# mikel-brostrom/boxmot

Measured on NVIDIA H100. Metric: tracker.update() frames/sec at 256 dets/frame, higher is better.
Workload: dtype bf16x3

## Files before the change

boxmot_b200/csrc/reid_tc.cuh:

```cuda
#pragma once
#include "wgmma.cuh"

namespace bmb {
namespace tcx {

typedef __nv_bfloat16 bf16;

__device__ __forceinline__ int tc_chunk_count(const int* d_n, int off, int cap) {
    int n = *d_n - off;
    n = n < 0 ? 0 : n;
    return n > cap ? cap : n;
}
using um::mbar_arrive;

__global__ void k_maxpool_planes(const float* __restrict__ in, int H, int W, int C, const int* __restrict__ d_n, int off,
                                 int cap, bf16* __restrict__ out_hi, bf16* __restrict__ out_lo) {
    const int n_crops = tc_chunk_count(d_n, off, cap);
    const int OH = H / 2, OW = W / 2, C8 = C / 8;
    const size_t total = (size_t)n_crops * C8 * OH * OW;
    for (size_t e = (size_t)blockIdx.x * blockDim.x + threadIdx.x; e < total; e += (size_t)gridDim.x * blockDim.x) {
        const int ox = (int)(e % OW);
        size_t r = e / OW;
        const int oy = (int)(r % OH); r /= OH;
        const int c8 = (int)(r % C8);
// ... 334 lines not shown
        }
        if (last && CP > CR) {
            constexpr int PP = (CP - CR) / 8;
            static_assert((CP - CR) % 8 == 0, "channel padding must be whole planes");
            for (int e = threadIdx.x; e < PP * rows_lv * W; e += 256) {
                const int pl = e / (rows_lv * W), r = e - pl * (rows_lv * W);
                const size_t o = (((size_t)n * (4 * C8) + br * C8 + CR / 8 + pl) * H + ya) * W + r;
                reinterpret_cast<uint4*>(a.y_hi)[o] = make_uint4(0u, 0u, 0u, 0u);
                reinterpret_cast<uint4*>(a.y_lo)[o] = make_uint4(0u, 0u, 0u, 0u);
            }
        }
        um::fence_async_smem();
        __syncthreads();
        TCK();
    }
#ifdef BMB_TC_CLOCKS
    if (threadIdx.x == 0 && blockIdx.x == 1 && n == 5) {
        printf("chain CP%d W%d br%d: setup %lld tma %lld |", CP, W, br, ck[1] - ck[0], ck[2] - ck[1]);
        for (int i = 2; i + 3 < nck + 1 && i + 3 <= 23; i += 3)
            printf(" wait %lld mma %lld dw %lld |", ck[i + 1] - ck[i], ck[i + 2] - ck[i + 1], ck[i + 3] - ck[i + 2]);
        printf(" total %lld\n", ck[nck - 1] - ck[0]);
    }
#endif
    if (threadIdx.x < act)
        *reinterpret_cast<float4*>(sP + (threadIdx.x / C4) * CR + (threadIdx.x % C4) * 4) = psum;
    __syncthreads();
    for (int c = threadIdx.x; c < CP; c += 256) {
        float s = 0.f;
        if (c < CR)
            for (int g = 0; g < n_grp; ++g) s += sP[g * CR + c];
        a.sums[br][((size_t)n * gridDim.x + tile) * CP + c] = s;
    }
    __threadfence();
    __syncthreads();
    __shared__ int s_last;
    __shared__ float s_mean[128], s_hid[16], s_gate[128];
    if (threadIdx.x == 0) {
        const int total = (int)gridDim.x * 4;
        const int prev = atomicAdd(a.gate.arrivals + n, 1);
        s_last = prev == total - 1;
        if (s_last) a.gate.arrivals[n] = 0;
    }
    __syncthreads();
    if (s_last) {
        __threadfence();
        gates_fold<256>(a.gate, n, s_mean, s_hid, s_gate);
    }
}

#ifndef BMB_S2_NS
#define BMB_S2_NS 0
#endif
#ifndef BMB_S3_R
#define BMB_S3_R 16
#endif
#ifndef BMB_S3_NS
#define BMB_S3_NS 0
#endif
#ifndef BMB_S4_NS
#define BMB_S4_NS 0
#endif
#define BMB_CHAIN_S2 16, 16, 32, 16, BMB_S2_NS
#define BMB_CHAIN_S3 32, 24, 16, BMB_S3_R, BMB_S3_NS
#define BMB_CHAIN_S4 32, 32, 8, 16, BMB_S4_NS
template <int CP, int CR, int W, int R, int NSPLIT>
inline cudaError_t chain_prepare() {
    return cudaFuncSetAttribute(k_chain_tc<CP, CR, W, R, NSPLIT>, cudaFuncAttributeMaxDynamicSharedMemorySize, (int)ChainGeom<CP, CR, W, R>::SMEM);
}
template <int CP, int CR, int W, int R, int NSPLIT>
inline void chain_launch(const ChainTcArgs& a, int tiles, int crops, const int* d_n, int off, cudaStream_t st) {
    k_chain_tc<CP, CR, W, R, NSPLIT><<<dim3(tiles, 4, crops), 256, ChainGeom<CP, CR, W, R>::SMEM, st>>>(a, d_n, off, crops);
}
template <int CP, int CR, int W, int R, int NSPLIT>
constexpr int chain_rows() { return R; }

constexpr int GEMM_THREADS = 288;

struct GemmTcArgs {
    CUtensorMap map_hi[2], map_lo[2];
    int src_planes[2];
    int src_kc[2];
    int n_src;
    int rows_per_tile;
    int tiles_per_crop, tiles_per_cta;
    int n_stage;
    const bf16* b_packed;
    int K8;
    int N, NP;
    const float* bias;
    int relu;
    const bf16* bfold;
    int midp, HW;
    int slot_bytes;
    bf16* out_hi; bf16* out_lo;
    float* out_f32;
    int pool;
    int pool2;
    int W;
    const bf16* b2_packed;
    const float* bias2;
    int N2, NP2;
    bf16* out2_hi; bf16* out2_lo;
    const float* head_w;
    const float* head_b;
    int head_feat;
};
struct GemmHeadIO {
    const CropDesc* crops;
    float* out;
    int out_ld;
};

struct GemmSmem {
    size_t b, b2, ring, a2, f, gate, total;
};
inline GemmSmem gemm_smem_layout(int K8, int NP, int NP2, int n_stage, bool tail, bool pool, int slot_bytes, bool pool2 = false) {
    GemmSmem s{};
    size_t o = 0;
    s.b = o; o += (size_t)K8 * 2 * NP * 16;
    s.b2 = o; if (tail) o += (size_t)(NP / 8) * 2 * NP2 * 16;
    o = (o + 127) & ~(size_t)127;
    s.ring = o; o += (size_t)n_stage * slot_bytes;
    s.a2 = o;
    if (tail) {
        size_t a2 = (size_t)2 * (NP / 8) * 128 * 16;
        if (pool2) a2 = a2 > (size_t)128 * (NP2 + 4) * 4 ? a2 : (size_t)128 * (NP2 + 4) * 4;
        o += a2;
    }
    s.f = pool2 ? s.a2 : o;
    if (pool) o += (size_t)128 * (NP + 4) * 4;
    s.gate = o; o += 4 * 32 * 4 + 64;
    s.total = o + 128;
    return s;
}

enum GemmMode { GM_PLAIN, GM_POOL, GM_TAIL, GM_TAIL_POOL2, GM_HEAD };

template <int NP, int NP2, int MODE>
constexpr int gemm_min_ctas() {
    return NP == 128 || ((MODE == GM_TAIL || MODE == GM_TAIL_POOL2) && NP >= 96) ? 1 : 2;
}

template <int NP, int NP2, int MODE>
__global__ void __launch_bounds__(GEMM_THREADS, (gemm_min_ctas<NP, NP2, MODE>()))
    k_gemm_tc(const __grid_constant__ GemmTcArgs a, const int* __restrict__ d_n, int off, int cap, const GemmSmem L, const GemmHeadIO hio) {
    constexpr bool tail = MODE == GM_TAIL || MODE == GM_TAIL_POOL2, pool = MODE == GM_POOL, pool2 = MODE == GM_TAIL_POOL2;
    static_assert(NP % 16 == 0 && NP >= 16 && NP <= 128, "NP: 16 .. 128 output channels");
    static_assert(tail ? (NP2 % 16 == 0 && NP2 >= 16 && NP2 <= 128) : NP2 == 0, "NP2: the tail's output channels");
    constexpr int NACC = (NP2 > NP ? NP2 : NP) / 2;
    const int n = blockIdx.y;
    if (n >= tc_chunk_count(d_n, off, cap)) return;
    extern __shared__ __align__(128) unsigned char smem[];
    __shared__ __align__(8) uint64_t bar_full[4], bar_empty[4], bar_w;
    const int warp = threadIdx.x >> 5, lane = threadIdx.x & 31;
    const int tile0 = blockIdx.x * a.tiles_per_cta;
    const int tile1 = min(tile0 + a.tiles_per_cta, a.tiles_per_crop);
    unsigned char* sB = smem + L.b;
    unsigned char* sB2 = smem + L.b2;
    unsigned char* sRing = smem + L.ring;
    unsigned char* sA2 = smem + L.a2;
    float* sF = reinterpret_cast<float*>(smem + L.f);

    if (threadIdx.x == 0) {
        for (int i = 0; i < a.n_stage; ++i) { um::mbar_init(&bar_full[i], 1); um::mbar_init(&bar_empty[i], 2); }
        um::mbar_init(&bar_w, 1);
        um::fence_mbar_init();
    }
    __syncthreads();

    if (warp == 8) {
        if (lane == 0) {
            {
                const uint32_t first = (uint32_t)((a.bfold ? 4 * a.midp : 0) / 8) * 2u * NP * 16u, total = (uint32_t)a.K8 * 2u * NP * 16u;
                const uint32_t b2 = tail ? (uint32_t)(NP / 8) * 2u * NP2 * 16u : 0u;
                um::mbar_expect_tx(&bar_w, total + b2);
                if (first) um::bulk_g2s(sB, reinterpret_cast<const unsigned char*>(a.bfold) + (size_t)n * first, first, &bar_w);
                if (total > first) um::bulk_g2s(sB + first, reinterpret_cast<const unsigned char*>(a.b_packed) + first, total - first, &bar_w);
                if (b2) um::bulk_g2s(sB2, a.b2_packed, b2, &bar_w);
            }
            uint32_t it = 0;
            for (int tile = tile0; tile < tile1; ++tile) {
                for (int s = 0; s < a.n_src; ++s) {
                    const int kc = a.src_kc[s];
                    for (int p0 = 0; p0 < a.src_planes[s]; p0 += kc, ++it) {
                        const uint32_t slot = it % (uint32_t)a.n_stage, ph = (it / (uint32_t)a.n_stage) & 1u;
                        um::mbar_wait(&bar_empty[slot], ph ^ 1u);
                        unsigned char* dst = sRing + (size_t)slot * a.slot_bytes;
                        um::mbar_expect_tx(&bar_full[slot], (uint32_t)kc * 128u * 16u * 2u);
                        um::tma_load_4d(dst, &a.map_hi[s], 0, tile * 2, p0, n, &bar_full[slot]);
                        um::tma_load_4d(dst + a.slot_bytes / 2, &a.map_lo[s], 0, tile * 2, p0, n, &bar_full[slot]);
                    }
                }
            }
        }
        return;
    }

    const int et = threadIdx.x;
    const int wg = warp >> 2;
    const int row = wg * 64 + (warp & 3) * 16 + (lane >> 2);
    const int cq = 2 * (lane & 3);
    const uint32_t lbo_b = 2u * NP * 16u, lo_off = (uint32_t)NP * 16u;
    um::mbar_wait(&bar_w, 0);
    float acc[NACC];
    uint32_t it = 0;
    for (int tile = tile0; tile < tile1; ++tile) {
        uint32_t kplane = 0, first = 1;
        uint32_t held = 0;
        for (int s = 0; s < a.n_src; ++s) {
            const int kc = a.src_kc[s];
            for (int p0 = 0; p0 < a.src_planes[s]; p0 += kc, ++it) {
                const uint32_t slot = it % (uint32_t)a.n_stage, ph = (it / (uint32_t)a.n_stage) & 1u;
                um::mbar_wait(&bar_full[slot], ph);
                const uint32_t ah = um::smem_u32(sRing + (size_t)slot * a.slot_bytes) + (uint32_t)wg * 1024u, al = ah + a.slot_bytes / 2;
                for (int ks = 0; ks < kc / 2; ++ks) {
                    const uint32_t bb = um::smem_u32(sB) + (kplane + 2 * ks) * lbo_b;
                    const uint64_t xh = um::make_desc(ah + ks * 2 * 2048u, 2048u, 128), xl = um::make_desc(al + ks * 2 * 2048u, 2048u, 128);
                    um::wg_fence();
                    um::mma<NP, false>(acc, xh, bb, lbo_b, 128, first ? 0u : 1u);
                    um::mma<NP, false>(acc, xl, bb, lbo_b, 128, 1u);
                    um::mma<NP, false>(acc, xh, bb + lo_off, lbo_b, 128, 1u);
                    first = 0;
                    um::wg_commit();
                    um::wg_wait<1>();
                    if (ks == 0 && kplane > 0 && (et & 127) == 0) mbar_arrive(&bar_empty[held]);
                }
                held = slot;
                kplane += kc;
            }
        }
        um::wg_wait<0>();
        um::wg_fence_acc<NACC>(acc);
        if ((et & 127) == 0) mbar_arrive(&bar_empty[held]);
        if constexpr (MODE == GM_HEAD) {
            um::bar_sync(1, 256);
            float* part = reinterpret_cast<float*>(sRing);
            float* pooled = part + 8 * NP;
            float* red = pooled + NP;
            float* feat = red + 8;
#pragma unroll
            for (int i = 0; i < NP / 8; ++i) {
                const int c = 8 * i + cq;
                const float2 b = *reinterpret_cast<const float2*>(a.bias + c);
                float o0 = fmaxf(acc[4 * i] + b.x, 0.f) + fmaxf(acc[4 * i + 2] + b.x, 0.f);
                float o1 = fmaxf(acc[4 * i + 1] + b.y, 0.f) + fmaxf(acc[4 * i + 3] + b.y, 0.f);
#pragma unroll
                for (int sh = 4; sh < 32; sh <<= 1) {
                    o0 += __shfl_xor_sync(0xffffffffu, o0, sh);
                    o1 += __shfl_xor_sync(0xffffffffu, o1, sh);
                }
                if (lane < 4) *reinterpret_cast<float2*>(part + warp * NP + c) = make_float2(o0, o1);
            }
            um::bar_sync(1, 256);
            for (int c = et; c < NP; c += 256)
                pooled[c] = (((part[c] + part[NP + c]) + (part[2 * NP + c] + part[3 * NP + c])) +
                             ((part[4 * NP + c] + part[5 * NP + c]) + (part[6 * NP + c] + part[7 * NP + c]))) / 128.f;
            um::bar_sync(1, 256);
            const int FEAT = a.head_feat, C = a.N;
            float sq = 0.f;
            for (int f = et; f < FEAT; f += 256) {
                float t[8] = {0.f, 0.f, 0.f, 0.f, 0.f, 0.f, 0.f, 0.f};
                int c = 0;
                for (; c + 8 <= C; c += 8) {
#pragma unroll
                    for (int u = 0; u < 8; ++u) t[u] = fmaf(pooled[c + u], a.head_w[(size_t)(c + u) * FEAT + f], t[u]);
                }
                for (; c < C; ++c) t[0] = fmaf(pooled[c], a.head_w[(size_t)c * FEAT + f], t[0]);
                float sv = a.head_b[f] + (((t[0] + t[1]) + (t[2] + t[3])) + ((t[4] + t[5]) + (t[6] + t[7])));
                sv = fmaxf(sv, 0.f);
                feat[f] = sv;
                sq = fmaf(sv, sv, sq);
            }
#pragma unroll
            for (int sh = 16; sh > 0; sh >>= 1) sq += __shfl_xor_sync(0xffffffffu, sq, sh);
            if (lane == 0) red[warp] = sq;
            um::bar_sync(1, 256);
            float tot = 0.f;
            for (int w = 0; w < 8; ++w) tot += red[w];
            const float nrm = sqrtf(tot);
            float* dst = hio.out + (size_t)hio.crops[off + n].out_row * hio.out_ld;
            for (int f = et; f < FEAT; f += 256) dst[f] = feat[f] / nrm;
            um::bar_sync(1, 256);
        } else {
#pragma unroll
            for (int i = 0; i < NP / 8; ++i) {
                const int c = 8 * i + cq;
                const float2 b = *reinterpret_cast<const float2*>(a.bias + c);
#pragma unroll
                for (int h = 0; h < 2; ++h) {
                    const int m = row + 8 * h, px = tile * 128 + m;
                    float o0 = acc[4 * i + 2 * h] + b.x, o1 = acc[4 * i + 2 * h + 1] + b.y;
                    if (a.relu) { o0 = fmaxf(o0, 0.f); o1 = fmaxf(o1, 0.f); }
                    if (a.out_f32) {
                        float* dst = a.out_f32 + ((size_t)n * a.HW + px) * a.N + c;
                        if (c + 1 < a.N) *reinterpret_cast<float2*>(dst) = make_float2(o0, o1);
                        else if (c < a.N) dst[0] = o0;
                    }
                    if constexpr (pool) {
                        *reinterpret_cast<float2*>(sF + (size_t)m * (NP + 4) + c) = make_float2(o0, o1);
                    } else if (a.out_hi || tail) {
                        uint32_t hv, lv;
                        um::split2(o0, o1, hv, lv);
                        if (a.out_hi) {
                            const size_t e = (((size_t)n * (NP / 8) + i) * a.HW + px) * 4 + (lane & 3);
                            reinterpret_cast<uint32_t*>(a.out_hi)[e] = hv;
                            reinterpret_cast<uint32_t*>(a.out_lo)[e] = lv;
                        }
                        if constexpr (tail) {
                            *reinterpret_cast<uint32_t*>(sA2 + ((size_t)i * 128 + m) * 16 + (lane & 3) * 4) = hv;
                            *reinterpret_cast<uint32_t*>(sA2 + ((size_t)(NP / 8 + i) * 128 + m) * 16 + (lane & 3) * 4) = lv;
                        }
                    }
                }
            }
            auto pool_store = [&](const int NPx, bf16* o_hi, bf16* o_lo) {
                um::bar_sync(1, 256);
                const int Wt = a.W, OW = Wt / 2, OHt = a.rows_per_tile / 2;
                const int items = OHt * OW * (NPx / 8);
                const int OHW = a.HW / 4;
                for (int e = et; e < items; e += 256) {
                    const int pp = e % (OHt * OW), c8 = e / (OHt * OW);
                    const int oy = pp / OW, ox = pp - oy * OW;
                    const float* f0 = sF + (size_t)((2 * oy) * Wt + 2 * ox) * (NPx + 4) + c8 * 8;
                    const float* f1 = f0 + (NPx + 4);
                    const float* f2 = f0 + (size_t)Wt * (NPx + 4);
                    const float* f3 = f2 + (NPx + 4);
                    uint32_t h[4], l[4];
#pragma unroll
                    for (int j = 0; j < 4; ++j) {
                        const float x0 = (f0[2 * j] + f1[2 * j] + f2[2 * j] + f3[2 * j]) * 0.25f;
                        const float x1 = (f0[2 * j + 1] + f1[2 * j + 1] + f2[2 * j + 1] + f3[2 * j + 1]) * 0.25f;
                        um::split2(x0, x1, h[j], l[j]);
                    }
                    const int opx = (tile * OHt + oy) * OW + ox;
                    const size_t o = ((size_t)n * (NPx / 8) + c8) * OHW + opx;
                    reinterpret_cast<uint4*>(o_hi)[o] = make_uint4(h[0], h[1], h[2], h[3]);
                    reinterpret_cast<uint4*>(o_lo)[o] = make_uint4(l[0], l[1], l[2], l[3]);
                }
                um::bar_sync(1, 256);
            };
            if constexpr (pool) pool_store(NP, a.out_hi, a.out_lo);
            if constexpr (tail) {
                um::fence_async_smem();
                um::bar_sync(2 + wg, 128);
                const uint32_t lbo_b2 = 2u * NP2 * 16u, lo2 = (uint32_t)NP2 * 16u;
                const uint32_t ah = um::smem_u32(sA2) + (uint32_t)wg * 1024u, al = ah + (uint32_t)(NP / 8) * 2048u;
                um::wg_fence();
                for (int ks = 0; ks < NP / 16; ++ks) {
                    const uint32_t bb = um::smem_u32(sB2) + ks * 2 * lbo_b2;
                    const uint64_t xh = um::make_desc(ah + ks * 2 * 2048u, 2048u, 128), xl = um::make_desc(al + ks * 2 * 2048u, 2048u, 128);
                    um::mma<NP2, false>(acc, xh, bb, lbo_b2, 128, ks > 0);
                    um::mma<NP2, false>(acc, xl, bb, lbo_b2, 128, 1u);
                    um::mma<NP2, false>(acc, xh, bb + lo2, lbo_b2, 128, 1u);
                }
                um::wg_commit();
                um::wg_wait<0>();
                um::wg_fence_acc<NACC>(acc);
                if constexpr (pool2) um::bar_sync(1, 256);
#pragma unroll
                for (int i = 0; i < NP2 / 8; ++i) {
                    const int c = 8 * i + cq;
                    const float2 b = *reinterpret_cast<const float2*>(a.bias2 + c);
#pragma unroll
                    for (int h = 0; h < 2; ++h) {
                        const int m = row + 8 * h, px = tile * 128 + m;
                        const float o0 = fmaxf(acc[4 * i + 2 * h] + b.x, 0.f), o1 = fmaxf(acc[4 * i + 2 * h + 1] + b.y, 0.f);
                        if constexpr (pool2) {
                            *reinterpret_cast<float2*>(sF + (size_t)m * (NP2 + 4) + c) = make_float2(o0, o1);
                        } else {
                            uint32_t hv, lv;
                            um::split2(o0, o1, hv, lv);
                            const size_t e = (((size_t)n * (NP2 / 8) + i) * a.HW + px) * 4 + (lane & 3);
                            reinterpret_cast<uint32_t*>(a.out2_hi)[e] = hv;
                            reinterpret_cast<uint32_t*>(a.out2_lo)[e] = lv;
                        }
                    }
                }
                if constexpr (pool2) pool_store(NP2, a.out2_hi, a.out2_lo);
            }
        }
    }
}

typedef void (*GemmKernel)(GemmTcArgs, const int*, int, int, GemmSmem, GemmHeadIO);
struct GemmInstance { int NP, NP2, mode; GemmKernel fn; };
#define BMB_GEMM(np, np2, mode) {np, np2, mode, k_gemm_tc<np, np2, mode>}
static const GemmInstance kGemmInstances[] = {
    BMB_GEMM(16, 0, GM_PLAIN), BMB_GEMM(32, 0, GM_PLAIN),
    BMB_GEMM(64, 0, GM_PLAIN), BMB_GEMM(96, 0, GM_PLAIN),
    BMB_GEMM(128, 0, GM_PLAIN),
    BMB_GEMM(64, 0, GM_POOL), BMB_GEMM(96, 0, GM_POOL),
    BMB_GEMM(64, 16, GM_TAIL), BMB_GEMM(96, 32, GM_TAIL), BMB_GEMM(128, 32, GM_TAIL),
    BMB_GEMM(64, 64, GM_TAIL_POOL2), BMB_GEMM(96, 96, GM_TAIL_POOL2),
    BMB_GEMM(128, 0, GM_HEAD),
};
#undef BMB_GEMM
inline GemmKernel gemm_instance(int NP, int NP2, int mode) {
    for (const GemmInstance& g : kGemmInstances)
        if (g.NP == NP && g.NP2 == NP2 && g.mode == mode) return g.fn;
    return nullptr;
}


struct FrontTcArgs {
    const uint8_t* images;
    size_t image_stride;
    int rows, cols;
    const void* crops;
    const bf16* w;
    const float* bias_tab;
    bf16* p_hi;
    bf16* p_lo;
    float* dbg_crop;
    int pad_mode;
};
struct FrontCrop { float x1, y1, x2, y2; int image, out_row; };

constexpr int FR_COLS = 39, FR_ROWS = 264, FR_CS = FR_ROWS * 8 + 16;
constexpr int FR_A_BYTES = FR_COLS * FR_CS;
constexpr int FR_W_BYTES = 7 * 4 * 32 * 16;
constexpr int FR_H_BYTES = 4 * 128 * 16 * 4;
constexpr size_t FR_SMEM = FR_A_BYTES + FR_W_BYTES + FR_H_BYTES + 128;

__device__ __forceinline__ void fr_coeff(int d, int src_n, double scale, bool clamp, int& idx, int& a0, int& a1) {
    float f = (float)(((double)d + 0.5) * scale - 0.5);
    int s = (int)floorf(f);
    f = f - (float)s;
    if (clamp) {
        if (s < 0) { s = 0; f = 0.f; }
        if (s >= src_n - 1) { s = src_n - 1; f = 0.f; }
    }
    idx = s;
    a0 = (int)rintf((1.0f - f) * 2048.0f);
    a1 = (int)rintf(f * 2048.0f);
}

__global__ void __launch_bounds__(256, 1) k_front_tc(const FrontTcArgs a, const int* __restrict__ d_n, int off, int cap) {
    const int n = blockIdx.y;
    if (n >= tc_chunk_count(d_n, off, cap)) return;
    const int strip = blockIdx.x;
    extern __shared__ __align__(128) unsigned char smem[];
    __shared__ int xi[128], xa0[128], xa1[128], yi[256], ya0[256], ya1[256];
    __shared__ __align__(16) float sBias[4 * 4 * 16];
    unsigned char* sA = smem;
    unsigned char* sW = smem + FR_A_BYTES;
    float* sH = reinterpret_cast<float*>(smem + FR_A_BYTES + FR_W_BYTES);
    const int warp = threadIdx.x >> 5, lane = threadIdx.x & 31;
    const FrontCrop cd = reinterpret_cast<const FrontCrop*>(a.crops)[off + n];
#ifdef BMB_TC_CLOCKS
    long long fk[16];
    int nfk = 0;
#define FCK() do { if (threadIdx.x == 0 && nfk < 16) fk[nfk++] = clock64(); } while (0)
#else
#define FCK() do { } while (0)
#endif
    FCK();

    const int x1 = (int)rintf(cd.x1), y1 = (int)rintf(cd.y1), x2 = (int)rintf(cd.x2), y2 = (int)rintf(cd.y2);
    const int cx1 = max(0, x1), cy1 = max(0, y1), cx2 = min(a.cols, x2), cy2 = min(a.rows, y2);
    const bool valid = cx2 > cx1 && cy2 > cy1;
    const int sw = cx2 - cx1, sh = cy2 - cy1;
    int nw = 128, nh = 256, pl = 0, pt = 0;
    if (valid && a.pad_mode) {
// ... 178 lines not shown
```

boxmot_b200/csrc/reid_tc_host.cuh:

```cuda
#pragma once
#include "reid_tc.cuh"

namespace bmb {

PFN_encodeTiled tensor_map_encoder() {
    static PFN_encodeTiled fn = nullptr;
    if (!fn) {
        void* p = nullptr;
        cudaDriverEntryPointQueryResult q;
        RCUDA_OK(cudaGetDriverEntryPoint("cuTensorMapEncodeTiled", &p, cudaEnableDefault, &q));
        if (!p) throw std::runtime_error("cuTensorMapEncodeTiled is not available in this driver");
        fn = (PFN_encodeTiled)p;
    }
    return fn;
}

static void encode_u32_map(CUtensorMap* out, const void* base, int rank, const cuuint64_t* dims, const cuuint64_t* strides,
                           const cuuint32_t* box) {
    cuuint32_t es[5] = {1, 1, 1, 1, 1};
    CUresult r = tensor_map_encoder()(out, CU_TENSOR_MAP_DATA_TYPE_UINT32, (cuuint32_t)rank, const_cast<void*>(base), dims, strides, box,
                                      es, CU_TENSOR_MAP_INTERLEAVE_NONE, CU_TENSOR_MAP_SWIZZLE_NONE, CU_TENSOR_MAP_L2_PROMOTION_L2_256B,
                                      CU_TENSOR_MAP_FLOAT_OOB_FILL_NONE);
    if (r != CUDA_SUCCESS) throw std::runtime_error("cuTensorMapEncodeTiled failed (" + std::to_string((int)r) + ")");
}
void make_rows_map(CUtensorMap* out, const void* base, int crops, int C8, int H, int W, int box_rows) {
    cuuint64_t dims[4] = {(cuuint64_t)W * 4, (cuuint64_t)H, (cuuint64_t)C8, (cuuint64_t)crops};
    cuuint64_t strides[3] = {(cuuint64_t)W * 16, (cuuint64_t)H * W * 16, (cuuint64_t)C8 * H * W * 16};
    cuuint32_t box[4] = {(cuuint32_t)(W + 2) * 4, (cuuint32_t)box_rows, (cuuint32_t)C8, 1};
    encode_u32_map(out, base, 4, dims, strides, box);
}
void make_tile_map(CUtensorMap* out, const void* base, int crops, int C8, int HW, int kc) {
    cuuint64_t dims[4] = {256, (cuuint64_t)HW / 64, (cuuint64_t)C8, (cuuint64_t)crops};
    cuuint64_t strides[3] = {1024, (cuuint64_t)HW * 16, (cuuint64_t)C8 * HW * 16};
    cuuint32_t box[4] = {256, 2, (cuuint32_t)kc, 1};
    encode_u32_map(out, base, 4, dims, strides, box);
}

namespace tcx {

inline uint16_t f2bf(float x) {
    uint32_t u;
    memcpy(&u, &x, 4);
    u += 0x7fffu + ((u >> 16) & 1u);
    return (uint16_t)(u >> 16);
}
inline float bf2f(uint16_t h) {
    const uint32_t u = (uint32_t)h << 16;
    float f;
    memcpy(&f, &u, 4);
    return f;
}
inline int pad16(int c) { return (c + 15) / 16 * 16; }

inline size_t pack_b(std::vector<uint16_t>& out, const float* w, int K, int N, int ldw, int K8, int NP, int k_row0 = 0,
                     bool identity = false) {
    size_t at = out.size();
    at = (at + 63) / 64 * 64;
    out.resize(at + (size_t)K8 * 2 * NP * 8, 0);
    for (int k = 0; k < K; ++k)
        for (int n = 0; n < N; ++n) {
            const float v = identity ? (k == n ? 1.f : 0.f) : w[(size_t)k * ldw + n];
            const uint16_t h = f2bf(v);
            const int kk = k_row0 + k;
            uint16_t* plane = out.data() + at + (size_t)(kk / 8) * 2 * NP * 8;
            plane[(size_t)n * 8 + kk % 8] = h;
            plane[(size_t)(NP + n) * 8 + kk % 8] = f2bf(v - bf2f(h));
        }
    return at;
}
inline size_t pack_f(std::vector<float>& out, const float* src, int n, int n_pad) {
    size_t at = (out.size() + 3) / 4 * 4;
    out.resize(at + n_pad, 0.f);
    for (int i = 0; i < n; ++i) out[at + i] = src[i];
    return at;
}

struct Planes {
    bf16* hi = nullptr;
    bf16* lo = nullptr;
};

enum LaunchKind { LK_CHAIN_S2, LK_CHAIN_S3, LK_CHAIN_S4, LK_GEMM, LK_MAXPOOL_PLANES, LK_GATES, LK_FRONT };
struct Launch {
    int kind = LK_GEMM;
    int cls = 0;
    ChainTcArgs chain{};
    int chain_tiles = 0;
    GemmTcArgs gemm{};
    const bf16* src_hi[2] = {nullptr, nullptr};
    const bf16* src_lo[2] = {nullptr, nullptr};
    FrontTcArgs front{};
    GemmSmem gl{};
    GemmKernel gemm_fn = nullptr;
    int gemm_ctas = 0;
    int gemm_groups = 0;
    int stage_after = -1;
    const bf16* dbg_hi = nullptr;
    const bf16* dbg_lo = nullptr;
    int dbg_C8 = 0, dbg_HW = 0, dbg_C = 0;
};

struct Plan {
    int chunk = 0;
    bool head_fused = false;
    bf16* d_wb = nullptr;
    float* d_wf = nullptr;
    Planes P, X1, Y, XA, XB;
    float* c5 = nullptr;
    float* sums[4] = {nullptr, nullptr, nullptr, nullptr};
    float* gates = nullptr;
    int* arrivals = nullptr;
    bf16* bfold = nullptr;
    float* dbg_crop = nullptr;
    float* dbg = nullptr;
    std::vector<Launch> launches;
    std::vector<Launch> launches_dbg;
    int smem_limit = 0;
};

inline void alloc_planes(Planes& p, size_t elems) {
    RCUDA_OK(cudaMalloc(&p.hi, elems * 2));
    RCUDA_OK(cudaMalloc(&p.lo, elems * 2));
}
inline void free_planes(Planes& p) {
    cudaFree(p.hi);
    cudaFree(p.lo);
    p.hi = p.lo = nullptr;
}

inline void plan_free(Plan* p) {
    if (!p) return;
    cudaFree(p->d_wb); cudaFree(p->d_wf); cudaFree(p->c5); cudaFree(p->dbg); cudaFree(p->gates); cudaFree(p->bfold); cudaFree(p->arrivals); cudaFree(p->dbg_crop);
    for (int b = 0; b < 4; ++b) cudaFree(p->sums[b]);
    free_planes(p->P); free_planes(p->X1); free_planes(p->Y); free_planes(p->XA); free_planes(p->XB);
    delete p;
}

}
}
```

boxmot_b200/csrc/reid_tc_plan.cuh:

```cuda
#pragma once

namespace bmb {
namespace tcx {

struct ChainShape { int CP, CR, W, H, R, kind; };
static const ChainShape kChainShapes[3] = {{16, 16, 32, 64, chain_rows<BMB_CHAIN_S2>(), LK_CHAIN_S2}, {32, 24, 16, 32, chain_rows<BMB_CHAIN_S3>(), LK_CHAIN_S3},
                                           {32, 32, 8, 16, chain_rows<BMB_CHAIN_S4>(), LK_CHAIN_S4}};

inline bool plan_supported(const ReidModel* m) {
    return m->arch == ARCH_OSNET && m->c[0] == 16 && m->c[1] == 64 && m->c[2] == 96 && m->c[3] == 128;
}

Plan* plan_build(ReidModel* m, const float* hw) {
    Plan* P = new Plan();
    try {
        P->chunk = m->chunk;
        const size_t CH = (size_t)m->chunk;
        int dev = 0;
        RCUDA_OK(cudaGetDevice(&dev));
        RCUDA_OK(cudaDeviceGetAttribute(&P->smem_limit, cudaDevAttrMaxSharedMemoryPerBlockOptin, dev));
        P->smem_limit -= 1024;
        alloc_planes(P->P, CH * 2048 * 16);
        alloc_planes(P->X1, CH * 2048 * 16);
        alloc_planes(P->Y, CH * 2048 * 64);
// ... 15 lines not shown
            const int midp = pad16(b.mid);
            for (int l = 0; l < 10; ++l) {
                bo[bi].pw[l] = pack_b(wb, hw + b.light[l].pw, b.mid, b.mid, b.mid, midp / 8, midp);
                size_t at = (wf.size() + 3) / 4 * 4;
                wf.resize(at + 9 * midp, 0.f);
                for (int t = 0; t < 9; ++t)
                    for (int c = 0; c < b.mid; ++c) wf[at + t * midp + c] = hw[b.light[l].dw + (size_t)t * b.mid + c];
                bo[bi].dw[l] = at;
                bo[bi].lb[l] = pack_f(wf, hw + b.light[l].b, b.mid, midp);
                if (bo[bi].lb[l] != at + (size_t)9 * midp) throw std::runtime_error("chain weights: taps and bias are not contiguous");
            }
            bo[bi].c1 = pack_b(wb, hw + b.c1w, b.cin, b.mid, b.mid, b.cin / 8, midp);
            bo[bi].c1b = pack_f(wf, hw + b.c1b, b.mid, midp);
            const int K8 = 4 * midp / 8 + b.cin / 8;
            if (b.has_ds)
                bo[bi].cx = pack_b(wb, hw + b.cw + (size_t)b.mid * b.cout, b.cin, b.cout, b.cout, K8, b.cout, 4 * midp);
            else
                bo[bi].cx = pack_b(wb, nullptr, b.cin, b.cout, b.cout, K8, b.cout, 4 * midp, true);
            bo[bi].cxb = pack_f(wf, hw + b.cb, b.cout, b.cout);
        }
        size_t tr[2], trb[2];
        for (int s = 0; s < 2; ++s) {
            const int C = m->c[s + 1];
            tr[s] = pack_b(wb, hw + m->trans_w[s], C, C, C, C / 8, C);
            trb[s] = pack_f(wf, hw + m->trans_b[s], C, C);
        }
        const size_t c5 = pack_b(wb, hw + m->c5w, m->c[3], m->c[3], m->c[3], m->c[3] / 8, m->c[3]);
        const size_t c5b = pack_f(wf, hw + m->c5b, m->c[3], m->c[3]);
        size_t fw, fb;
        {
            const double mean[3] = {0.485, 0.456, 0.406}, stdv[3] = {0.229, 0.224, 0.225};
            const int C0 = m->c[0];
            fw = (wb.size() + 63) / 64 * 64;
            wb.resize(fw + 7 * 4 * 32 * 8, 0);
            for (int kx = 0; kx < 7; ++kx)
                for (int ky = 0; ky < 7; ++ky)
                    for (int ci = 0; ci < 3; ++ci)
                        for (int co = 0; co < C0; ++co) {
                            const float v = (float)((double)hw[m->stem_w + (size_t)((ky * 7 + kx) * 3 + ci) * C0 + co] / (255.0 * stdv[ci]));
                            const int k = ky * 4 + ci;
                            uint16_t* plane = wb.data() + fw + ((size_t)(kx * 4 + k / 8) * 32) * 8;
                            const uint16_t h = f2bf(v);
                            plane[(size_t)co * 8 + k % 8] = h;
                            plane[(size_t)(16 + co) * 8 + k % 8] = f2bf(v - bf2f(h));
                        }
            fb = (wf.size() + 3) / 4 * 4;
            wf.resize(fb + 4 * 4 * 16, 0.f);
            const int lo_[4] = {3, 1, 0, 0}, hi_[4] = {6, 6, 6, 4};
            for (int rc = 0; rc < 4; ++rc)
                for (int cc = 0; cc < 4; ++cc)
                    for (int co = 0; co < C0; ++co) {
                        double acc = hw[m->stem_b + co];
                        for (int ky = lo_[rc]; ky <= hi_[rc]; ++ky)
                            for (int kx = lo_[cc]; kx <= hi_[cc]; ++kx)
                                for (int ci = 0; ci < 3; ++ci)
                                    acc -= (double)hw[m->stem_w + (size_t)((ky * 7 + kx) * 3 + ci) * C0 + co] * mean[ci] / stdv[ci];
                        wf[fb + (rc * 4 + cc) * 16 + co] = (float)acc;
                    }
        }
        RCUDA_OK(cudaMalloc(&P->d_wb, wb.size() * 2 + 256));
        RCUDA_OK(cudaMemcpy(P->d_wb, wb.data(), wb.size() * 2, cudaMemcpyHostToDevice));
        RCUDA_OK(cudaMalloc(&P->d_wf, wf.size() * 4 + 256));
        RCUDA_OK(cudaMemcpy(P->d_wf, wf.data(), wf.size() * 4, cudaMemcpyHostToDevice));
        const bf16* WB = P->d_wb;
        const float* WF = P->d_wf;
        const float* W32 = m->d_w;

        RCUDA_OK(chain_prepare<BMB_CHAIN_S2>());
        RCUDA_OK(chain_prepare<BMB_CHAIN_S3>());
        RCUDA_OK(chain_prepare<BMB_CHAIN_S4>());
        for (const GemmInstance& gi : kGemmInstances)
            RCUDA_OK(cudaFuncSetAttribute(gi.fn, cudaFuncAttributeMaxDynamicSharedMemorySize, P->smem_limit));
        RCUDA_OK(cudaFuncSetAttribute(k_front_tc, cudaFuncAttributeMaxDynamicSharedMemorySize, (int)FR_SMEM));

        struct Src { Planes* buf; int C8; };
        auto gemm = [&](int H, int Wd, std::vector<Src> srcs, size_t b_off, int N, size_t bias_off, bool relu) -> Launch {
            Launch L{};
            L.kind = LK_GEMM;
            L.cls = CLS_POINTWISE;
            GemmTcArgs& g = L.gemm;
            g.n_src = (int)srcs.size();
            g.rows_per_tile = 128 / Wd;
            g.tiles_per_crop = H * Wd / 128;
            g.tiles_per_cta = g.tiles_per_crop >= 16 ? 4 : (g.tiles_per_crop >= 4 ? 2 : 1);
            g.K8 = 0;
            for (int s = 0; s < g.n_src; ++s) {
                const int C8 = srcs[s].C8;
                const int kc = C8 % 4 == 0 ? 4 : 2;
                g.src_planes[s] = C8;
                g.src_kc[s] = kc;
                g.K8 += C8;
                L.src_hi[s] = srcs[s].buf->hi;
                L.src_lo[s] = srcs[s].buf->lo;
            }
            g.b_packed = WB + b_off;
            g.N = N;
            g.NP = pad16(N);
            g.bias = WF + bias_off;
            g.relu = relu ? 1 : 0;
            g.HW = H * Wd;
            g.W = Wd;
            return L;
        };
        auto finish_into = [&](Launch& L, std::vector<Launch>* out) {
            GemmTcArgs& g = L.gemm;
            const bool tail = g.b2_packed != nullptr;
            if (g.NP > 128 || (tail && g.NP2 > 128)) throw std::runtime_error("tensor-core GEMM: more than 128 output channels");
            const int mode = g.head_w ? GM_HEAD : g.pool ? GM_POOL : !tail ? GM_PLAIN : g.pool2 ? GM_TAIL_POOL2 : GM_TAIL;
            L.gemm_fn = gemm_instance(g.NP, tail ? g.NP2 : 0, mode);
            if (!L.gemm_fn)
                throw std::runtime_error("tensor-core GEMM: no kernel instance for NP = " + std::to_string(g.NP) + ", NP2 = " +
                                         std::to_string(tail ? g.NP2 : 0) + ", epilogue mode " + std::to_string(mode));
            auto layout = [&](int ns) { return gemm_smem_layout(g.K8, g.NP, g.NP2, ns, tail, g.pool != 0, g.slot_bytes, g.pool2 != 0); };
            auto ctas = [&](int ns) {
                const size_t bytes = layout(ns).total;
                int c = 0;
                if ((int)bytes <= P->smem_limit)
                    RCUDA_OK(cudaOccupancyMaxActiveBlocksPerMultiprocessor(&c, L.gemm_fn, GEMM_THREADS, bytes));
                return c;
            };
            int ns = 0;
            for (int pass = 0; pass < 2 && !ns; ++pass) {
                int kc_max = 2;
                for (int s = 0; s < g.n_src; ++s) {
                    if (pass == 1) g.src_kc[s] = 2;
                    kc_max = std::max(kc_max, g.src_kc[s]);
                }
                g.slot_bytes = kc_max * 128 * 16 * 2;
                for (int cand = 4; cand >= 2 && !ns; --cand)
                    if (ctas(cand) >= 2) ns = cand;
            }
            if (!ns) {
                int kc_max = 2;
                for (int s = 0; s < g.n_src; ++s) {
                    g.src_kc[s] = g.src_planes[s] % 4 == 0 ? 4 : 2;
                    kc_max = std::max(kc_max, g.src_kc[s]);
                }
                g.slot_bytes = kc_max * 128 * 16 * 2;
                for (int cand = 4; cand >= 2 && !ns; --cand)
                    if (ctas(cand) >= 1) ns = cand;
            }
            if (!ns) throw std::runtime_error("tensor-core GEMM does not fit shared memory");
            L.gemm_ctas = ctas(ns);
            for (int s = 0; s < g.n_src; ++s) {
                make_tile_map(&g.map_hi[s], L.src_hi[s], P->chunk, g.src_planes[s], g.HW, g.src_kc[s]);
                make_tile_map(&g.map_lo[s], L.src_lo[s], P->chunk, g.src_planes[s], g.HW, g.src_kc[s]);
            }
            L.gl = layout(ns);
            g.n_stage = ns;
            L.gemm_groups = (g.tiles_per_crop + g.tiles_per_cta - 1) / g.tiles_per_cta;
            out->push_back(L);
        };
        auto dbg = [&](Launch& L, int stage, const Planes& buf, int C8, int HW, int C) {
            L.stage_after = stage;
            L.dbg_hi = buf.hi; L.dbg_lo = buf.lo; L.dbg_C8 = C8; L.dbg_HW = HW; L.dbg_C = C;
        };

        auto build_launches = [&](bool fuse_trans, std::vector<Launch>* out) {
            auto finish = [&](Launch& L) { finish_into(L, out); };
        {
            Launch L{};
            L.kind = LK_FRONT;
            L.cls = CLS_STEM;
            L.front.w = WB + fw;
            L.front.bias_tab = WF + fb;
            L.front.p_hi = P->P.hi; L.front.p_lo = P->P.lo;
            dbg(L, 2, P->P, 2, 2048, 16);
            out->push_back(L);
        }
        Planes* X = &P->P;
        Planes* Xo = &P->XA;
        Planes* Xspare = &P->XB;
        int xC8 = 2;
        int H = 64, Wd = 32;
        int stage = 3;
        {
            const BlockW& b = m->blocks[0];
            Launch L = gemm(H, Wd, {{X, xC8}}, bo[0].c1, b.mid, bo[0].c1b, true);
            L.gemm.out_hi = P->X1.hi; L.gemm.out_lo = P->X1.lo;
            dbg(L, 100, P->X1, pad16(b.mid) / 8, H * Wd, pad16(b.mid));
            finish(L);
        }
        for (int s = 0; s < 3; ++s) {
            const ChainShape& cs = kChainShapes[s];
            bool trans_done = false;
            for (int j = 0; j < 2; ++j) {
                const int bi = s * 2 + j;
                const BlockW& b = m->blocks[bi];
                const int midp = pad16(b.mid);
                {
                    Launch L{};
                    L.kind = cs.kind;
                    L.cls = CLS_LIGHTCONV;
                    ChainTcArgs& c = L.chain;
                    make_rows_map(&c.map_hi, P->X1.hi, P->chunk, midp / 8, H, Wd, cs.R + 8);
                    make_rows_map(&c.map_lo, P->X1.lo, P->chunk, midp / 8, H, Wd, cs.R + 8);
                    for (int l = 0; l < 10; ++l) {
                        c.wpw[l] = WB + bo[bi].pw[l];
                        c.wdw[l] = WF + bo[bi].dw[l];
                        c.bias[l] = WF + bo[bi].lb[l];
                    }
                    c.y_hi = P->Y.hi; c.y_lo = P->Y.lo;
                    for (int br = 0; br < 4; ++br) c.sums[br] = P->sums[br];
                    c.H = H;
                    GatesTcArgs& ga = c.gate;
                    for (int br = 0; br < 4; ++br) ga.sums[br] = P->sums[br];
                    ga.g1w = W32 + b.g1w; ga.g1b = W32 + b.g1b; ga.g2w = W32 + b.g2w; ga.g2b = W32 + b.g2b;
                    ga.gates = P->gates;
                    ga.mid = b.mid; ga.midp = midp; ga.hid = b.hid; ga.tiles = H / cs.R; ga.HW = H * Wd;
                    ga.w3 = W32 + b.cw; ga.bfold = P->bfold; ga.N = b.cout; ga.NP = pad16(b.cout);
                    ga.arrivals = P->arrivals;
                    L.chain_tiles = H / cs.R;
                    dbg(L, 200 + bi, P->Y, 4 * midp / 8, H * Wd, 4 * midp);
                    out->push_back(L);
                }
                {
                    Launch L = gemm(H, Wd, {{&P->Y, 4 * midp / 8}, {X, xC8}}, bo[bi].cx, b.cout, bo[bi].cxb, true);
                    GemmTcArgs& g = L.gemm;
                    g.bfold = P->bfold;
                    g.midp = midp;
                    g.out_hi = Xo->hi; g.out_lo = Xo->lo;
                    bool fused_trans = false;
                    if (j == 0) {
                        const BlockW& nb = m->blocks[bi + 1];
                        const int nmidp = pad16(nb.mid);
                        const GemmSmem probe = gemm_smem_layout(g.K8, g.NP, nmidp, 2, true, false, 4 * 128 * 16 * 2);
                        if ((int)probe.total <= P->smem_limit) {
                            g.b2_packed = WB + bo[bi + 1].c1;
                            g.bias2 = WF + bo[bi + 1].c1b;
                            g.N2 = nb.mid; g.NP2 = nmidp;
                            g.out2_hi = P->X1.hi; g.out2_lo = P->X1.lo;
                        }
                    } else if (s < 2 && fuse_trans) {
// ... 23 lines not shown
                    if (j == 0 && !fused_next) {
                        const BlockW& nb = m->blocks[bi + 1];
                        Launch L2 = gemm(H, Wd, {{X, xC8}}, bo[bi + 1].c1, nb.mid, bo[bi + 1].c1b, true);
                        L2.gemm.out_hi = P->X1.hi; L2.gemm.out_lo = P->X1.lo;
                        dbg(L2, 100 + bi + 1, P->X1, pad16(nb.mid) / 8, H * Wd, pad16(nb.mid));
                        finish(L2);
                    }
                }
            }
            if (s < 2) {
                const int C = m->c[s + 1];
                if (!trans_done) {
                    Launch L = gemm(H, Wd, {{X, xC8}}, tr[s], C, trb[s], true);
                    L.gemm.pool = 1;
                    L.gemm.out_hi = Xo->hi; L.gemm.out_lo = Xo->lo;
                    dbg(L, stage++, *Xo, C / 8, H * Wd / 4, C);
                    finish(L);
                    Planes* t = X; X = Xo; Xo = t;
                }
                H /= 2; Wd /= 2;
                const BlockW& nb = m->blocks[(s + 1) * 2];
                Launch L = gemm(H, Wd, {{X, xC8}}, bo[(s + 1) * 2].c1, nb.mid, bo[(s + 1) * 2].c1b, true);
                L.gemm.out_hi = P->X1.hi; L.gemm.out_lo = P->X1.lo;
                dbg(L, 100 + (s + 1) * 2, P->X1, pad16(nb.mid) / 8, H * Wd, pad16(nb.mid));
                finish(L);
            }
        }
        {
            Launch L = gemm(H, Wd, {{X, xC8}}, c5, m->c[3], c5b, true);
            if (fuse_trans && H * Wd == 128) {
                L.gemm.head_w = W32 + m->fcw;
                L.gemm.head_b = W32 + m->fcb;
                L.gemm.head_feat = m->feat;
                L.cls = CLS_HEAD;
                P->head_fused = true;
            } else {
                L.gemm.out_f32 = P->c5;
            }
            L.stage_after = 11;
            finish(L);
        }
        };
        build_launches(true, &P->launches);
        build_launches(false, &P->launches_dbg);
    } catch (...) {
        plan_free(P);
        throw;
    }
    return P;
}

struct FrontInput { const uint8_t* images; size_t image_stride; int rows, cols; const CropDesc* crops; float* out; int out_ld; };

template <class Prof>
bool plan_run(ReidModel* m, const FrontInput& fi, const int* d_n, int off, int upper, cudaStream_t st, Prof& prof) {
    Plan* P = m->tc;
    for (const Launch& L : (m->debug_stop >= 0 ? P->launches_dbg : P->launches)) {
        prof.begin(L.cls);
        switch (L.kind) {
            case LK_FRONT: {
                FrontTcArgs fa = L.front;
                fa.images = fi.images; fa.image_stride = fi.image_stride; fa.rows = fi.rows; fa.cols = fi.cols; fa.crops = fi.crops;
                fa.pad_mode = m->preprocess;
                if (m->debug_stop == 50) {
                    if (!P->dbg_crop) RCUDA_OK(cudaMalloc(&P->dbg_crop, sizeof(float) * (size_t)P->chunk * 256 * 128 * 3));
                    fa.dbg_crop = P->dbg_crop;
                }
                k_front_tc<<<dim3(4, upper), 256, FR_SMEM, st>>>(fa, d_n, off, upper);
                break;
            }
            case LK_MAXPOOL_PLANES:
                k_maxpool_planes<<<m->sms * 4, 256, 0, st>>>(m->bufA, 128, 64, m->c[0], d_n, off, upper, P->P.hi, P->P.lo);
                break;
            case LK_CHAIN_S2:
                chain_launch<BMB_CHAIN_S2>(L.chain, L.chain_tiles, upper, d_n, off, st);
                break;
            case LK_CHAIN_S3:
                chain_launch<BMB_CHAIN_S3>(L.chain, L.chain_tiles, upper, d_n, off, st);
                break;
            case LK_CHAIN_S4:
                chain_launch<BMB_CHAIN_S4>(L.chain, L.chain_tiles, upper, d_n, off, st);
                break;
            case LK_GEMM:
                L.gemm_fn<<<dim3(L.gemm_groups, upper), GEMM_THREADS, L.gl.total, st>>>(L.gemm, d_n, off, upper, L.gl, GemmHeadIO{fi.crops, fi.out, fi.out_ld});
                break;
        }
        prof.end();
        if (m->debug_stop == 50 && L.kind == LK_FRONT) {
            m->debug_ptr = P->dbg_crop;
            m->debug_floats_per_crop = (size_t)256 * 128 * 3;
            return true;
        }
        if (m->debug_stop >= 0 && L.stage_after == m->debug_stop) {
            if (L.stage_after == 11) {
                m->debug_ptr = P->c5;
                m->debug_floats_per_crop = (size_t)128 * m->c[3];
            } else {
                k_planes_to_nhwc<<<m->sms * 4, 256, 0, st>>>(L.dbg_hi, L.dbg_lo, L.dbg_C8, L.dbg_HW, L.dbg_C, d_n, off, upper, P->dbg);
                m->debug_ptr = P->dbg;
                m->debug_floats_per_crop = (size_t)L.dbg_HW * L.dbg_C;
            }
            return true;
        }
    }
    return false;
}

}
}
```

Measured before the change: 703.8.

## Make tensor-core GEMM persistent with balanced tile split and double-buffered fold weights

The GEMM launch changes from a per-crop grid of tile groups to a persistent grid sized to resident CTAs. Each CTA takes a contiguous, evenly balanced range of (crop, tile) items, and the per-crop gate-folded weight rows are reloaded into a double-buffered shared region whenever the crop changes, guarded by new mbarriers. The head epilogue now uses the held ring slot as scratch and releases it only after finishing. The intent is to remove tail imbalance and launch-shape waste when the number of crops is small or uneven, at the cost of extra barrier traffic, fold reloads and added shared memory, which may reduce occupancy.

```diff
diff --git a/boxmot_b200/csrc/reid_tc.cuh b/boxmot_b200/csrc/reid_tc.cuh
--- a/boxmot_b200/csrc/reid_tc.cuh
+++ b/boxmot_b200/csrc/reid_tc.cuh
@@ -440,8 +440,10 @@
     int src_kc[2];
     int n_src;
     int rows_per_tile;
-    int tiles_per_crop, tiles_per_cta;
+    int tiles_per_crop;
+    int tiles_per_cta;
     int n_stage;
+    int n_fold;
     const bf16* b_packed;
     int K8;
     int N, NP;
@@ -470,13 +472,15 @@
 };
 
 struct GemmSmem {
-    size_t b, b2, ring, a2, f, gate, total;
+    size_t b, b2, fold, ring, a2, f, gate, total;
 };
-inline GemmSmem gemm_smem_layout(int K8, int NP, int NP2, int n_stage, bool tail, bool pool, int slot_bytes, bool pool2 = false) {
+inline GemmSmem gemm_smem_layout(int K8, int NP, int NP2, int n_stage, bool tail, bool pool, int slot_bytes, bool pool2 = false,
+                                 int fold_planes2 = 0) {
     GemmSmem s{};
     size_t o = 0;
     s.b = o; o += (size_t)K8 * 2 * NP * 16;
     s.b2 = o; if (tail) o += (size_t)(NP / 8) * 2 * NP2 * 16;
+    s.fold = o; o += (size_t)fold_planes2 * 2 * NP * 16;
     o = (o + 127) & ~(size_t)127;
     s.ring = o; o += (size_t)n_stage * slot_bytes;
     s.a2 = o;
@@ -506,22 +510,28 @@
     static_assert(NP % 16 == 0 && NP >= 16 && NP <= 128, "NP: 16 .. 128 output channels");
     static_assert(tail ? (NP2 % 16 == 0 && NP2 >= 16 && NP2 <= 128) : NP2 == 0, "NP2: the tail's output channels");
     constexpr int NACC = (NP2 > NP ? NP2 : NP) / 2;
-    const int n = blockIdx.y;
-    if (n >= tc_chunk_count(d_n, off, cap)) return;
+    const int tpc = a.tiles_per_crop;
+    const int items = tc_chunk_count(d_n, off, cap) * tpc;
+    const int cta = (int)(blockIdx.y * gridDim.x + blockIdx.x), n_cta = (int)(gridDim.x * gridDim.y);
+    const int q = items / n_cta, r = items - q * n_cta;
+    const int item0 = cta * q + min(cta, r);
+    const int n_items = q + (cta < r ? 1 : 0);
+    if (n_items == 0) return;
     extern __shared__ __align__(128) unsigned char smem[];
-    __shared__ __align__(8) uint64_t bar_full[4], bar_empty[4], bar_w;
+    __shared__ __align__(8) uint64_t bar_full[4], bar_empty[4], bar_w, bar_fold_full[2], bar_fold_empty[2];
     const int warp = threadIdx.x >> 5, lane = threadIdx.x & 31;
-    const int tile0 = blockIdx.x * a.tiles_per_cta;
-    const int tile1 = min(tile0 + a.tiles_per_cta, a.tiles_per_crop);
     unsigned char* sB = smem + L.b;
     unsigned char* sB2 = smem + L.b2;
     unsigned char* sRing = smem + L.ring;
     unsigned char* sA2 = smem + L.a2;
     float* sF = reinterpret_cast<float*>(smem + L.f);
+    const uint32_t fold_planes = a.bfold ? (uint32_t)(4 * a.midp / 8) : 0u, fold_bytes = fold_planes * 2u * NP * 16u;
+    const uint32_t fold_step = a.n_fold > 1 ? 1u : 0u;
 
     if (threadIdx.x == 0) {
         for (int i = 0; i < a.n_stage; ++i) { um::mbar_init(&bar_full[i], 1); um::mbar_init(&bar_empty[i], 2); }
         um::mbar_init(&bar_w, 1);
+        for (int i = 0; i < 2; ++i) { um::mbar_init(&bar_fold_full[i], 1); um::mbar_init(&bar_fold_empty[i], 2); }
         um::fence_mbar_init();
     }
     __syncthreads();
@@ -529,15 +539,24 @@
     if (warp == 8) {
         if (lane == 0) {
             {
-                const uint32_t first = (uint32_t)((a.bfold ? 4 * a.midp : 0) / 8) * 2u * NP * 16u, total = (uint32_t)a.K8 * 2u * NP * 16u;
+                const uint32_t total = (uint32_t)a.K8 * 2u * NP * 16u;
                 const uint32_t b2 = tail ? (uint32_t)(NP / 8) * 2u * NP2 * 16u : 0u;
-                um::mbar_expect_tx(&bar_w, total + b2);
-                if (first) um::bulk_g2s(sB, reinterpret_cast<const unsigned char*>(a.bfold) + (size_t)n * first, first, &bar_w);
-                if (total > first) um::bulk_g2s(sB + first, reinterpret_cast<const unsigned char*>(a.b_packed) + first, total - first, &bar_w);
+                um::mbar_expect_tx(&bar_w, total - fold_bytes + b2);
+                if (total > fold_bytes)
+                    um::bulk_g2s(sB + fold_bytes, reinterpret_cast<const unsigned char*>(a.b_packed) + fold_bytes, total - fold_bytes, &bar_w);
                 if (b2) um::bulk_g2s(sB2, a.b2_packed, b2, &bar_w);
             }
-            uint32_t it = 0;
-            for (int tile = tile0; tile < tile1; ++tile) {
+            uint32_t it = 0, fb = fold_step, fph = 3u;
+            int n = item0 / tpc, tile = item0 - n * tpc;
+            for (int left = n_items; left > 0; --left) {
+                if (fold_bytes && (left == n_items || tile == 0)) {
+                    fb ^= fold_step;
+                    um::mbar_wait(&bar_fold_empty[fb], (fph >> fb) & 1u);
+                    fph ^= 1u << fb;
+                    um::mbar_expect_tx(&bar_fold_full[fb], fold_bytes);
+                    um::bulk_g2s(fb ? smem + L.fold : sB, reinterpret_cast<const unsigned char*>(a.bfold) + (size_t)n * fold_bytes,
+                                 fold_bytes, &bar_fold_full[fb]);
+                }
                 for (int s = 0; s < a.n_src; ++s) {
                     const int kc = a.src_kc[s];
                     for (int p0 = 0; p0 < a.src_planes[s]; p0 += kc, ++it) {
@@ -549,6 +568,7 @@
                         um::tma_load_4d(dst + a.slot_bytes / 2, &a.map_lo[s], 0, tile * 2, p0, n, &bar_full[slot]);
                     }
                 }
+                if (++tile == tpc) { tile = 0; ++n; }
             }
         }
         return;
@@ -561,8 +581,14 @@
     const uint32_t lbo_b = 2u * NP * 16u, lo_off = (uint32_t)NP * 16u;
     um::mbar_wait(&bar_w, 0);
     float acc[NACC];
-    uint32_t it = 0;
-    for (int tile = tile0; tile < tile1; ++tile) {
+    uint32_t it = 0, fb = fold_step, fph = 0u;
+    int n = item0 / tpc, tile = item0 - n * tpc;
+    for (int left = n_items; left > 0; --left) {
+        if (fold_bytes && (left == n_items || tile == 0)) {
+            fb ^= fold_step;
+            um::mbar_wait(&bar_fold_full[fb], (fph >> fb) & 1u);
+            fph ^= 1u << fb;
+        }
         uint32_t kplane = 0, first = 1;
         uint32_t held = 0;
         for (int s = 0; s < a.n_src; ++s) {
@@ -571,8 +597,9 @@
                 const uint32_t slot = it % (uint32_t)a.n_stage, ph = (it / (uint32_t)a.n_stage) & 1u;
                 um::mbar_wait(&bar_full[slot], ph);
                 const uint32_t ah = um::smem_u32(sRing + (size_t)slot * a.slot_bytes) + (uint32_t)wg * 1024u, al = ah + a.slot_bytes / 2;
+                const uint32_t bbase = um::smem_u32(kplane < fold_planes && fb ? smem + L.fold : sB);
                 for (int ks = 0; ks < kc / 2; ++ks) {
-                    const uint32_t bb = um::smem_u32(sB) + (kplane + 2 * ks) * lbo_b;
+                    const uint32_t bb = bbase + (kplane + 2 * ks) * lbo_b;
                     const uint64_t xh = um::make_desc(ah + ks * 2 * 2048u, 2048u, 128), xl = um::make_desc(al + ks * 2 * 2048u, 2048u, 128);
                     um::wg_fence();
                     um::mma<NP, false>(acc, xh, bb, lbo_b, 128, first ? 0u : 1u);
@@ -589,10 +616,13 @@
         }
         um::wg_wait<0>();
         um::wg_fence_acc<NACC>(acc);
-        if ((et & 127) == 0) mbar_arrive(&bar_empty[held]);
+        if ((et & 127) == 0) {
+            if constexpr (MODE != GM_HEAD) mbar_arrive(&bar_empty[held]);
+            if (fold_bytes && (left == 1 || tile + 1 == tpc)) mbar_arrive(&bar_fold_empty[fb]);
+        }
         if constexpr (MODE == GM_HEAD) {
             um::bar_sync(1, 256);
-            float* part = reinterpret_cast<float*>(sRing);
+            float* part = reinterpret_cast<float*>(sRing + (size_t)held * a.slot_bytes);
             float* pooled = part + 8 * NP;
             float* red = pooled + NP;
             float* feat = red + 8;
@@ -638,7 +668,9 @@
             const float nrm = sqrtf(tot);
             float* dst = hio.out + (size_t)hio.crops[off + n].out_row * hio.out_ld;
             for (int f = et; f < FEAT; f += 256) dst[f] = feat[f] / nrm;
+            um::fence_async_smem();
             um::bar_sync(1, 256);
+            if ((et & 127) == 0) mbar_arrive(&bar_empty[held]);
         } else {
 #pragma unroll
             for (int i = 0; i < NP / 8; ++i) {
@@ -737,6 +769,7 @@
                 if constexpr (pool2) pool_store(NP2, a.out2_hi, a.out2_lo);
             }
         }
+        if (++tile == tpc) { tile = 0; ++n; }
     }
 }
 
diff --git a/boxmot_b200/csrc/reid_tc_host.cuh b/boxmot_b200/csrc/reid_tc_host.cuh
--- a/boxmot_b200/csrc/reid_tc_host.cuh
+++ b/boxmot_b200/csrc/reid_tc_host.cuh
@@ -93,7 +93,7 @@
     GemmSmem gl{};
     GemmKernel gemm_fn = nullptr;
     int gemm_ctas = 0;
-    int gemm_groups = 0;
+    int gemm_grid = 0;
     int stage_after = -1;
     const bf16* dbg_hi = nullptr;
     const bf16* dbg_lo = nullptr;
diff --git a/boxmot_b200/csrc/reid_tc_plan.cuh b/boxmot_b200/csrc/reid_tc_plan.cuh
--- a/boxmot_b200/csrc/reid_tc_plan.cuh
+++ b/boxmot_b200/csrc/reid_tc_plan.cuh
@@ -121,7 +121,6 @@
             g.n_src = (int)srcs.size();
             g.rows_per_tile = 128 / Wd;
             g.tiles_per_crop = H * Wd / 128;
-            g.tiles_per_cta = g.tiles_per_crop >= 16 ? 4 : (g.tiles_per_crop >= 4 ? 2 : 1);
             g.K8 = 0;
             for (int s = 0; s < g.n_src; ++s) {
                 const int C8 = srcs[s].C8;
@@ -150,15 +149,25 @@
             if (!L.gemm_fn)
                 throw std::runtime_error("tensor-core GEMM: no kernel instance for NP = " + std::to_string(g.NP) + ", NP2 = " +
                                          std::to_string(tail ? g.NP2 : 0) + ", epilogue mode " + std::to_string(mode));
-            auto layout = [&](int ns) { return gemm_smem_layout(g.K8, g.NP, g.NP2, ns, tail, g.pool != 0, g.slot_bytes, g.pool2 != 0); };
-            auto ctas = [&](int ns) {
-                const size_t bytes = layout(ns).total;
+            const int fold_planes = g.bfold ? 4 * g.midp / 8 : 0;
+            if (fold_planes && (g.n_src != 2 || g.src_planes[0] != fold_planes))
+                throw std::runtime_error("tensor-core GEMM: the gate-folded rows must be the whole first source");
+            auto layout = [&](int ns, int nf) {
+                return gemm_smem_layout(g.K8, g.NP, g.NP2, ns, tail, g.pool != 0, g.slot_bytes, g.pool2 != 0, nf == 2 ? fold_planes : 0);
+            };
+            auto ctas = [&](int ns, int nf) {
+                const size_t bytes = layout(ns, nf).total;
                 int c = 0;
                 if ((int)bytes <= P->smem_limit)
                     RCUDA_OK(cudaOccupancyMaxActiveBlocksPerMultiprocessor(&c, L.gemm_fn, GEMM_THREADS, bytes));
                 return c;
             };
-            int ns = 0;
+            int ns = 0, nf = 1;
+            auto pick = [&](int min_ctas) {
+                for (int cand = 4; cand >= 2 && !ns; --cand)
+                    for (int f = fold_planes ? 2 : 1; f >= 1 && !ns; --f)
+                        if (ctas(cand, f) >= min_ctas) { ns = cand; nf = f; }
+            };
             for (int pass = 0; pass < 2 && !ns; ++pass) {
                 int kc_max = 2;
                 for (int s = 0; s < g.n_src; ++s) {
@@ -166,8 +175,7 @@
                     kc_max = std::max(kc_max, g.src_kc[s]);
                 }
                 g.slot_bytes = kc_max * 128 * 16 * 2;
-                for (int cand = 4; cand >= 2 && !ns; --cand)
-                    if (ctas(cand) >= 2) ns = cand;
+                pick(2);
             }
             if (!ns) {
                 int kc_max = 2;
@@ -176,18 +184,20 @@
                     kc_max = std::max(kc_max, g.src_kc[s]);
                 }
                 g.slot_bytes = kc_max * 128 * 16 * 2;
-                for (int cand = 4; cand >= 2 && !ns; --cand)
-                    if (ctas(cand) >= 1) ns = cand;
+                pick(1);
             }
             if (!ns) throw std::runtime_error("tensor-core GEMM does not fit shared memory");
-            L.gemm_ctas = ctas(ns);
+            if (g.head_w && (9 * g.NP + 8 + g.head_feat) * 4 > g.slot_bytes)
+                throw std::runtime_error("tensor-core GEMM: the head's scratch does not fit a ring slot");
+            L.gemm_ctas = ctas(ns, nf);
             for (int s = 0; s < g.n_src; ++s) {
                 make_tile_map(&g.map_hi[s], L.src_hi[s], P->chunk, g.src_planes[s], g.HW, g.src_kc[s]);
                 make_tile_map(&g.map_lo[s], L.src_lo[s], P->chunk, g.src_planes[s], g.HW, g.src_kc[s]);
             }
-            L.gl = layout(ns);
+            L.gl = layout(ns, nf);
             g.n_stage = ns;
-            L.gemm_groups = (g.tiles_per_crop + g.tiles_per_cta - 1) / g.tiles_per_cta;
+            g.n_fold = nf;
+            L.gemm_grid = L.gemm_ctas * m->sms;
             out->push_back(L);
         };
         auto dbg = [&](Launch& L, int stage, const Planes& buf, int C8, int HW, int C) {
@@ -377,7 +387,7 @@
                 chain_launch<BMB_CHAIN_S4>(L.chain, L.chain_tiles, upper, d_n, off, st);
                 break;
             case LK_GEMM:
-                L.gemm_fn<<<dim3(L.gemm_groups, upper), GEMM_THREADS, L.gl.total, st>>>(L.gemm, d_n, off, upper, L.gl, GemmHeadIO{fi.crops, fi.out, fi.out_ld});
+                L.gemm_fn<<<std::min(upper * L.gemm.tiles_per_crop, L.gemm_grid), GEMM_THREADS, L.gl.total, st>>>(L.gemm, d_n, off, upper, L.gl, GemmHeadIO{fi.crops, fi.out, fi.out_ld});
                 break;
         }
         prof.end();
```

Result: no change. 711.1 (median of 6 runs) (+1.0%).
